# UoL-SignalProcessingGroup/SMC-NUTS

Hardware: AMD Instinct MI355X
Metric: leapfrog-steps/sec (higher is better)
Workload: dtype f64

## Files before the change

include/smcnuts_hip.h:

```cpp
#ifndef SMCNUTS_HIP_H
#define SMCNUTS_HIP_H

#include <stddef.h>
#include <stdint.h>

#ifdef __cplusplus
extern "C" {
#endif

typedef struct smcn_ctx smcn_ctx;

#define SMCN_MODEL_GAUSS 0
#define SMCN_MODEL_ARMA 1
#define SMCN_MODEL_PRMWCD 2
#define SMCN_MODEL_HOST 3
#define SMCN_MODEL_GLM 4
#define SMCN_MODEL_HGLM 5
#define SMCN_MODEL_CATEGORICAL 6
#define SMCN_MODEL_ORDINAL 7

#define SMCN_LKERNEL_FORWARD 0
#define SMCN_LKERNEL_GAUSSIAN 1

#define SMCN_FLAG_TAPE_OVERFLOW 1
// ... 17 lines not shown
int smcn_get_proposal(smcn_ctx* ctx, double* r, double* x_new, double* r_new, double* logw_new);
int smcn_set_momentum(smcn_ctx* ctx, const double* r);
int smcn_set_proposal(smcn_ctx* ctx, const double* r, const double* x_new, const double* r_new);

int smcn_target_eval(smcn_ctx* ctx, const double* x, int64_t M, double phi, double* logp,
                     double* grad, double* lpri, double* llik);
int smcn_target_constrain(smcn_ctx* ctx, const double* x, int64_t M, double* out);

int smcn_init_particles_std_normal(smcn_ctx* ctx, double phi);
int smcn_init_weights(smcn_ctx* ctx, double phi, const double* logq0);

int smcn_normalise_partials(smcn_ctx* ctx, double out[4]);
int smcn_normalise_apply(smcn_ctx* ctx, double loglik);
int smcn_normalise(smcn_ctx* ctx, double* loglik, double* ess);

int smcn_moment_sums(smcn_ctx* ctx, const double* mean_or_null, double* sums);

int smcn_resample_multinomial(smcn_ctx* ctx, const double* u, double loglik, double log_n_total,
                              int64_t iteration, int64_t* idx_out);
#define SMCN_RESAMPLE_MULTINOMIAL 0
#define SMCN_RESAMPLE_SYSTEMATIC 1
int smcn_set_resample_scheme(smcn_ctx* ctx, int scheme);
int smcn_set_wide_eval(smcn_ctx* ctx, int on);
int smcn_set_lane_grid(smcn_ctx* ctx, int64_t waves);
int smcn_set_lane_segments(smcn_ctx* ctx, int segments);

int smcn_set_nuts_cap(smcn_ctx* ctx, int doublings, int widen);
int smcn_nuts_parked(smcn_ctx* ctx, int64_t* parked);
int smcn_set_nuts_requeue(smcn_ctx* ctx, int doublings);

int smcn_propose_nuts(smcn_ctx* ctx, double step_size, double phi, int max_depth, double delta_max,
                      int64_t iteration, const double* tape, const int64_t* tape_off);
int smcn_get_tree_stats(smcn_ctx* ctx, int32_t* nleap, int32_t* depth, int32_t* ndraws, int32_t* flags);
int smcn_last_leapfrogs(smcn_ctx* ctx, int64_t* total);
int smcn_get_density_parts(smcn_ctx* ctx, double* lpri0, double* llik0, double* lpri1, double* llik1);

int smcn_reweight(smcn_ctx* ctx, int lkernel);
int smcn_accept_reject(smcn_ctx* ctx, double phi, const double* u, int64_t iteration);
int smcn_reweight_asymptotic(smcn_ctx* ctx, double phi_old, double phi_new);
int smcn_set_logw_density_ratio(smcn_ctx* ctx, double phi_num, double phi_den);

int smcn_set_lkernel_values(smcn_ctx* ctx, const double* L, const double* q);

int smcn_gauss_lkernel_sums(smcn_ctx* ctx, const double* shift, double* sums);
int smcn_gauss_lkernel_logpdf(smcn_ctx* ctx, const double* mu_x, const double* m0, const double* B,
                              const double* U, double c0);
// ... 114 lines not shown
```

smcnuts_amd/_capi.py:

```python
import ctypes as C
import os

import numpy as np

from . import build as _build

MODEL_GAUSS, MODEL_ARMA, MODEL_PRMWCD, MODEL_HOST = 0, 1, 2, 3
MODEL_GLM = 4
MODEL_HGLM = 5
MODEL_CATEGORICAL = 6
MODEL_ORDINAL = 7
HOST_TARGET_FN = C.CFUNCTYPE(C.c_int, C.c_void_p, C.c_int64, C.c_int, C.POINTER(C.c_double), C.c_int,
                             C.POINTER(C.c_double), C.POINTER(C.c_double), C.POINTER(C.c_double),
                             C.POINTER(C.c_double))
LKERNEL_FORWARD, LKERNEL_GAUSSIAN = 0, 1

_dp = C.POINTER(C.c_double)
_ip = C.POINTER(C.c_int32)
_lp = C.POINTER(C.c_int64)
_ctx = C.c_void_p

SIGNATURES = {
    "smcn_version": ([], C.c_int),
    "smcn_last_error": ([_ctx], C.c_char_p),
# ... 39 lines not shown
    "smcn_temper_partials": ([_ctx, C.c_double, C.c_double, _dp], C.c_int),
    "smcn_temper_bisect": ([_ctx, C.c_double, C.c_double, C.POINTER(C.c_double), C.POINTER(C.c_int)], C.c_int),
    "smcn_temper_bisect_pass": ([_ctx, C.c_int, C.c_double], C.c_int),
    "smcn_temper_bisect_buffers": ([_ctx, C.c_int, C.POINTER(C.c_void_p), C.POINTER(C.c_void_p)], C.c_int),
    "smcn_temper_bisect_decide": ([_ctx, C.c_int, C.c_int, C.c_double, C.c_double], C.c_int),
    "smcn_temper_bisect_result": ([_ctx, C.POINTER(C.c_double), C.POINTER(C.c_int)], C.c_int),
    "smcn_eval_proposed_parts": ([_ctx, C.c_int], C.c_int),
    "smcn_commit": ([_ctx, _lp], C.c_int),
    "smcn_fast_begin": ([_ctx, C.c_int64, C.c_int, C.c_int], C.c_int),
    "smcn_fast_buffers": ([_ctx, C.POINTER(C.c_void_p), C.POINTER(C.c_void_p), C.POINTER(C.c_int)], C.c_int),
    "smcn_set_resample_uniforms": ([_ctx, _dp], C.c_int),
    "smcn_step_begin": ([_ctx, C.c_int64], C.c_int),
    "smcn_step_finish": ([_ctx, C.c_int64, C.c_int, C.c_int, C.c_double, C.c_double, C.c_double, C.c_int,
                          C.c_double, C.c_int, C.c_int, _dp, _lp], C.c_int),
    "smcn_fast_read": ([_ctx, _dp, _dp, _dp], C.c_int),
    "smcn_fast_read_from": ([_ctx, _dp, _dp, _dp, C.c_int64], C.c_int),
    "smcn_history_download": ([_ctx, C.c_int64, C.c_int64, _dp, _dp], C.c_int),
    "smcn_fuse_begin": ([_ctx, C.c_int, C.c_int], C.c_int),
    "smcn_fuse_buffers": ([_ctx, C.POINTER(C.c_void_p), C.POINTER(C.c_void_p), C.POINTER(C.c_int)], C.c_int),
    "smcn_fuse_run": ([_ctx, C.c_int64, C.c_int, C.c_int, C.c_int, C.c_double, C.c_double, C.c_double, C.c_int,
                       C.c_double, C.c_int], C.c_int),
    "smcn_set_resample_scheme": ([_ctx, C.c_int], C.c_int),
    "smcn_set_wide_eval": ([_ctx, C.c_int], C.c_int),
    "smcn_set_lane_grid": ([_ctx, C.c_int64], C.c_int),
    "smcn_set_lane_segments": ([_ctx, C.c_int], C.c_int),
    "smcn_set_host_target": ([_ctx, HOST_TARGET_FN, C.c_void_p], C.c_int),
    "smcn_moment_sums_of": ([_ctx, _dp, C.c_int, _dp, _dp], C.c_int),
    "smcn_block_resample_local": ([_ctx, C.c_int64], C.c_int),
    "smcn_block_launch": ([_ctx, C.c_int64, C.c_int, C.c_double, C.c_double, C.c_int, C.c_double], C.c_int),
    "smcn_block_post": ([_ctx, C.c_int64, C.c_int, C.c_int], C.c_int),
    "smcn_block_partials_get": ([_ctx, C.c_int, _dp], C.c_int),
    "smcn_block_partials_set": ([_ctx, C.c_int, C.c_int, _dp], C.c_int),
    "smcn_block_stats": ([_ctx, C.c_int64, C.c_int, C.c_int, C.c_int, C.c_double, C.c_double, C.c_int], C.c_int),
    "smcn_block_wait": ([_ctx, C.c_int, C.POINTER(C.c_int), C.POINTER(C.c_int)], C.c_int),
    "smcn_block_commit": ([_ctx, C.c_int64, C.c_int], C.c_int),
    "smcn_block_ess": ([_ctx, C.c_int, _dp], C.c_int),
    "smcn_fuse_decide": ([_ctx, C.c_int64, C.c_int, C.c_int, C.c_double, C.c_double, C.POINTER(C.c_int)], C.c_int),
    "smcn_fuse_finish": ([_ctx, C.c_int64, C.c_int, C.c_int, C.c_int, C.c_double, C.c_double,
                          C.POINTER(C.c_int)], C.c_int),
    "smcn_partials_get": ([_ctx, _dp], C.c_int),
    "smcn_partials_set_gathered": ([_ctx, _dp, C.c_int], C.c_int),
    "smcn_timers": ([_ctx, _dp, C.c_int], C.c_int),
    "smcn_selftest_math": ([_ctx, _dp, C.c_int64, _dp], C.c_int),
    "smcn_measure_peaks": ([_ctx, _dp], C.c_int),
    "smcn_selftest_wide": ([_ctx, C.c_int, _dp, C.c_int64, _dp], C.c_int),
    "smcn_device_cache_trim": ([C.c_int, C.POINTER(C.c_int64), C.POINTER(C.c_int64)], C.c_int),
# ... 343 lines not shown
```

smcnuts_amd/csrc/smcn_api.hip:

```cpp
#include <hip/hip_runtime.h>

#include <dlfcn.h>

#include <cmath>
#include <cstdio>
#include <cstring>
#include <chrono>
#include <cstdlib>
#include <map>
#include <mutex>
#include <string>
#include <thread>
#include <unordered_map>
#include <vector>

#include "../../include/smcnuts_hip.h"
#include "smcn_nuts.hpp"
#include "smcn_nuts_wave.hpp"
#include "smcn_nuts_fin.hpp"
#include "smcn_nuts2.hpp"
#include "smcn_nuts3.hpp"
#include "smcn_temper.hpp"
#include "smcn_nuts_host.hpp"
#include "smcn_weights.hpp"
#include "smcn_glk.hpp"
#include "smcn_step.hpp"
#include "smcn_comm.hpp"
#include "smcn_pointwise.hpp"
#include "smcn_predict.hpp"
#include "smcn_predict_draws.hpp"

using namespace smcn;

namespace {
struct Roctx {
    int (*push)(const char*) = nullptr;
    int (*pop)() = nullptr;
    Roctx() {
        void* h = dlopen("librocprofiler-sdk-roctx.so", RTLD_LAZY | RTLD_GLOBAL);
        if (!h) h = dlopen("libroctx64.so", RTLD_LAZY | RTLD_GLOBAL);
        if (h) {
            push = (int (*)(const char*))dlsym(h, "roctxRangePushA");
            pop = (int (*)())dlsym(h, "roctxRangePop");
        }
    }
};
inline Roctx& roctx() { static Roctx r; return r; }
struct Range {
    explicit Range(const char* name) { if (roctx().push && roctx().pop) roctx().push(name); }
    ~Range() { if (roctx().push && roctx().pop) roctx().pop(); }
    Range(const Range&) = delete;
};
thread_local std::string g_create_error;
constexpr int kMaxPart = 1024;
constexpr int kTimerRing = 512;
// ... 43 lines not shown
    bool kin_valid = false;
    bool r_pm = false, r_new_pm = false;
    unsigned long long* prof = nullptr;
    double* tape_d = nullptr;
    int64_t* tape_off_d = nullptr;
    int64_t tape_cap = 0;
    bool momentum_set = false, lg_set = false, q_set = false, u_set = false;
    double *hist = nullptr, *ss = nullptr, *lp = nullptr, *gath = nullptr, *hist_x = nullptr, *hist_logw = nullptr;
    double* u_res = nullptr;
    double *in_rec = nullptr, *out_rec = nullptr;
    double* nuts_scratch = nullptr;
    int64_t nuts_scratch_len = 0;
    int64_t fast_K = -1;
    bool fast_hist = false;
    int fuse_max = 0;
    int64_t rec_cap = 0;
    int resample_scheme = 0;
    bool fused_ok = false;
    bool lane_kernel = false;
    int64_t arma_T = 0;
    double *tb_state = nullptr, *tb_part = nullptr, *tb_local = nullptr, *tb_gath = nullptr;
    int tb_world = 0, tb_blocks = 0;
    int wide_eval = 1;
    int64_t lane_grid_cap = 0;
    int lane_segments = 0;
    unsigned long long* handover = nullptr;
    int64_t handover_len = 0;
    bool plain_block = false;
    ncclComm_t comm = nullptr;
    int comm_rank = 0, comm_world = 1;
    double *g_ttot_all = nullptr, *g_toff_all = nullptr, *g_keys = nullptr, *g_keys_send = nullptr, *g_keys_recv = nullptr,
           *g_rows_send = nullptr, *g_rows_recv = nullptr;
    int32_t *g_dest = nullptr, *g_order = nullptr;
    int64_t g_serve_cap = 0;
    int g_world = 0;
    smcn_host_target_fn host_fn = nullptr;
    void* host_user = nullptr;
    double *hc_vec = nullptr, *hc_sc = nullptr, *hc_gp = nullptr, *hc_gl = nullptr;
    int32_t* hc_st = nullptr;
    std::vector<double> hx, hlp, hll, hgp, hgl;
    double* n2_ovf = nullptr;
    int64_t n2_ovf_len = 0;
    double* ss_scratch = nullptr;
    double* rows_h = nullptr;
    double* hist_h = nullptr;
    bool hist_h_valid = false;
// ... 732 lines not shown
    HIPC(c, stream_wait(c->stream));
    if (c->own_stream && c->stream) pool_give(c->device, c->stream);
    c->stream = (hipStream_t)s;
    c->own_stream = false;
    return 0;
}

int smcn_synchronize(smcn_ctx* c) {
    CHECK_CTX(c);
    HIPC(c, stream_wait(c->stream));
    return 0;
}

int smcn_set_resample_scheme(smcn_ctx* c, int scheme) {
    CHECK_CTX(c);
    if (scheme != 0 && scheme != 1) FAIL(c, "smcn_set_resample_scheme: 0 (multinomial) or 1 (systematic)");
    c->resample_scheme = scheme;
    return 0;
}
int smcn_set_wide_eval(smcn_ctx* c, int on) {
    CHECK_CTX(c);
    if (on != 0 && on != 1) FAIL(c, "smcn_set_wide_eval: 0 or 1");
    c->wide_eval = on;
    return 0;
}

int smcn_set_lane_grid(smcn_ctx* c, int64_t waves) {
    CHECK_CTX(c);
    c->lane_grid_cap = waves;
    return 0;
}

int smcn_set_lane_segments(smcn_ctx* c, int segments) {
    CHECK_CTX(c);
    if (segments < 0 || segments > 64) FAIL(c, "smcn_set_lane_segments: 0 (auto) .. 64");
    c->lane_segments = segments;
    return 0;
}

int smcn_set_host_target(smcn_ctx* c, smcn_host_target_fn fn, void* user) {
    CHECK_CTX(c);
    if (c->model != SMCN_MODEL_HOST) FAIL(c, "smcn_set_host_target: the context was not created with SMCN_MODEL_HOST");
    c->host_fn = fn;
    c->host_user = user;
    return 0;
}
// ... 784 lines not shown
        c->in_rec = c->out_rec = nullptr;
        HIPC(c, dalloc(&c->in_rec, N * cap * n2_in_doubles(D)));
        HIPC(c, dalloc(&c->out_rec, N * cap * n2_out_doubles(D)));
        c->rec_cap = cap;
    }
    const size_t lds = (size_t)n3_lds_bytes<Model>(LC, LF);
    int64_t blocks = (N + kN3Block - 1) / kN3Block;
    const int64_t resident = (int64_t)c->num_cu * 4;
    if (c->lane_grid_cap > 0 && blocks > c->lane_grid_cap) blocks = c->lane_grid_cap;
    else if (c->lane_grid_cap == 0 && blocks > resident) blocks = resident;
    if (((N + blocks - 1) / blocks + 63) / 64 > kN3ReadyWords) blocks = (N + kN3Block - 1) / kN3Block;
    if (int rc = grow_scratch(c, c->n2_ovf, c->n2_ovf_len, blocks * kN3Block * 2 * (int64_t)n3_ovf_pairs(D, LC, LF))) return rc;
    a.ovf = c->n2_ovf;
    if (phase != 2) {
        if (c->momentum_set && B != 1) FAIL(c, "nuts3: caller-supplied momenta go with single transitions");
        nuts3_prep_kernel<D><<<grid_for(N * B, 256), 256, 0, c->stream>>>(c->x, c->momentum_set ? c->r : nullptr, c->r,
                                                                         c->in_rec, N, c->base, c->seed, a.iter, B, tape_d,
                                                                         tape_off_d);
        c->momentum_set = false;
        a.in = c->in_rec;
        a.out = c->out_rec;
        a.B = B;
        a.logw0 = (fuse_reweight && B > 1) ? c->logw : nullptr;
        a.wide = (c->wide_eval ? 1 : 0) | 2;
        const bool queued = blocks * kN3Block < N;
        a.seg_len = 0;
        a.seg_tail = 0;
        a.seg_align = 4;
        if (queued) {
            const int64_t per_wave = (N + blocks - 1) / blocks, words = (per_wave + 63) / 64;
            int nseg = c->lane_segments > 0 ? c->lane_segments : 4;
            if (nseg > B) nseg = (int)B;
            while (nseg > 1 && nseg * words > kN3ReadyWords) --nseg;
            a.seg_tail = 0;
            if (nseg > 1) a.seg_len = (int)((B + nseg - 1) / nseg);
            int64_t segs = a.seg_len > 0 ? (B + a.seg_len - 1) / a.seg_len : 1;
            const int64_t last_len = B - (segs - 1) * a.seg_len;
            if (segs > 1 && last_len >= 2 && (segs + 1) * words <= kN3ReadyWords) {
                a.seg_tail = (int)((2 * last_len + 2) / 5 > 0 ? (2 * last_len + 2) / 5 : 1);
                ++segs;
            }
            const int64_t hw = N * (segs - 1) * 2 * (n2_vp(D) / 2 + 1);
            if (hw > c->handover_len) {
                HIPC(c, stream_wait(c->stream));
                if (c->handover) (void)cached_free(c->handover);
                c->handover = nullptr;
                HIPC(c, cached_malloc((void**)&c->handover, sizeof(unsigned long long) * (size_t)hw));
// ... 1966 lines not shown
```

smcnuts_amd/csrc/smcn_nuts3.hpp:

```cpp
#pragma once
#include "smcn_nuts2.hpp"
#include <type_traits>

namespace smcn {

constexpr int kN3Block = 64;
constexpr int kN3ReadyWords = 64;


__constant__ double kArmaFinishTab[24] = {
    1.4426950408889634074, 6.93147180369123816490e-01, 1.90821492927058770002e-10,
    2.08767569878680989792e-09, 2.50521083854417187751e-08, 2.75573192239858906526e-07,
    2.75573192239858906526e-06, 2.48015873015873015873e-05, 1.98412698412698412698e-04,
    1.38888888888888888889e-03, 8.33333333333333333333e-03, 4.16666666666666666667e-02,
    1.66666666666666666667e-01,
    0.70710678118654752440,
    9.52380952380952380952e-02, 1.05263157894736842105e-01, 1.17647058823529411765e-01,
    1.33333333333333333333e-01, 1.53846153846153846154e-01, 1.81818181818181818182e-01,
    2.22222222222222222222e-01, 2.85714285714285714286e-01, 4.0e-01, 6.66666666666666666667e-01};

struct ArmaLaneModel {
    static constexpr int D = 4;
    static constexpr bool HAS_WIDE = true;
    using cptr = const __attribute__((address_space(4))) double*;
// ... 186 lines not shown
        else if constexpr (A >= 8) return dpp_mov<0x110 + K>(v);
        else return dpp_mov<(K == 1) ? 0x90 : 0x44>(v);
    }
    template <int CTRL, int ROWS>
    static __device__ __forceinline__ double row_join(double v, double fill) { return dpp_fill<CTRL, ROWS>(v, fill); }
    template <class F>
    static __device__ __forceinline__ void seg_walk(const double* Yp, int S, bool extra, F&& step) {
        const int nfull = (S - 1) >> 2, rem = (S - 1) & 3;
        double yp = Yp[0];
        double c0 = Yp[1], c1 = Yp[2], c2 = Yp[3], c3 = Yp[4];
        const double* q = Yp + 5;
        for (int c = 0; c < nfull; ++c) {
            const double n0 = q[0], n1 = q[1], n2 = q[2], n3 = q[3];
            q += 4;
            step(yp, c0); step(c0, c1); step(c1, c2); step(c2, c3);
            yp = c3;
            c0 = n0; c1 = n1; c2 = n2; c3 = n3;
        }
        if (rem > 0) { step(yp, c0); yp = c0; c0 = c1; c1 = c2; c2 = c3; }
        if (rem > 1) { step(yp, c0); yp = c0; c0 = c1; c1 = c2; }
        if (rem > 2) { step(yp, c0); yp = c0; c0 = c1; }
        if (extra) step(yp, c0);
    }
    template <int A>
    __device__ __forceinline__ void recur_wide(const double (&x)[4], bool act, unsigned long long mask, const double* Yl,
                                               double __attribute__((ext_vector_type(2)))* XCH, int lane, double& ss_o,
                                               double& gm_o, double& gb_o, double& gt_o) const {
        using d2 = double __attribute__((ext_vector_type(2)));
        const int rank = (int)__builtin_amdgcn_mbcnt_hi((unsigned)(mask >> 32), __builtin_amdgcn_mbcnt_lo((unsigned)mask, 0u));
        if (act) {
            d2 t;
            t.x = x[0]; t.y = x[1];
            XCH[2 * rank] = t;
            t.x = x[2]; t.y = x[3];
            XCH[2 * rank + 1] = t;
        }
        wave_exchange_fence();
        const int g = lane / A, a = lane % A;
        const d2 q0 = XCH[2 * g], q1 = XCH[2 * g + 1];
        const double mu = q0.x, beta = q0.y, theta = q1.x;
        const double nth = -theta, nbeta = -beta;
        const int n = T - 1, S = (n + A - 1) / A, R = n - A * (S - 1);
        const bool extra = a < R;
        const int i0 = 1 + a * (S - 1) + (a < R ? a : R);
        const bool first = a == 0;
        const double y0 = Yl[0];
        const double e_init = fma(nbeta, mu, y0 - mu), dm_init = -(1.0 + beta), db_init = -mu;
        double e = first ? e_init : 0.0, dm = first ? dm_init : 0.0, db = first ? db_init : 0.0, dt = 0.0;
        auto state_step = [&](double yp, double yt) __attribute__((always_inline)) {
            dt = fma(nth, dt, -e);
            dm = fma(nth, dm, -1.0);
            db = fma(nth, db, -yp);
            e = fma(nth, e, fma(nbeta, yp, yt - mu));
        };
        seg_walk(Yl + (i0 - 1), S, extra, state_step);
        double pm = 1.0;
        {
            double base = nth;
            for (int m = S - 2; m > 0; m >>= 1) {
                pm = (m & 1) ? pm * base : pm;
                base = base * base;
            }
        }
// ... 24 lines not shown
                if constexpr (A >= 32) return dpp_mov<0x138>(v);
                else return seg_shift<A, 1>(v, 0.0);
            };
            const double ei = prev(E), mi = prev(M), bi = prev(Bv), ti = prev(Tt);
            e = first ? e_init : ei;
            dm = first ? dm_init : mi;
            db = first ? db_init : bi;
            dt = first ? 0.0 : ti;
        }
        double ss = first ? e * e : 0.0, gm = first ? e * dm : 0.0, gb = first ? e * db : 0.0, gt = 0.0;
        auto full_step = [&](double yp, double yt) __attribute__((always_inline)) {
            dt = fma(nth, dt, -e);
            dm = fma(nth, dm, -1.0);
            db = fma(nth, db, -yp);
            e = fma(nth, e, fma(nbeta, yp, yt - mu));
            ss = fma(e, e, ss);
            gm = fma(e, dm, gm);
            gb = fma(e, db, gb);
            gt = fma(e, dt, gt);
        };
        seg_walk(Yl + (i0 - 1), S, extra, full_step);
        if constexpr (A == 64) wave_sum4(ss, gm, gb, gt, ss, gm, gb, gt);
        else { ss = group_sum<A>(ss); gm = group_sum<A>(gm); gb = group_sum<A>(gb); gt = group_sum<A>(gt); }
        if (first) {
            d2 t;
            t.x = ss; t.y = gm;
            XCH[2 * g] = t;
            t.x = gb; t.y = gt;
            XCH[2 * g + 1] = t;
        }
        wave_exchange_fence();
        if (act) {
            const d2 r0 = XCH[2 * rank], r1 = XCH[2 * rank + 1];
            ss_o = r0.x; gm_o = r0.y; gb_o = r1.x; gt_o = r1.y;
        }
    }
};

template <class Model>
__global__ void __launch_bounds__(256) lane_eval_kernel(const double* mdata, const double* x, int64_t M, int64_t rs,
                                                        int64_t cs, double phi, double* logp, double* grad, int64_t grs,
                                                        int64_t gcs, double* lpri_o, double* llik_o) {
    constexpr int D = Model::D;
    Model model;
    model.init(mdata);
    for (int64_t i = (int64_t)blockIdx.x * blockDim.x + threadIdx.x; i < M; i += (int64_t)gridDim.x * blockDim.x) {
// ... 59 lines not shown

__device__ __forceinline__ bool compact_mode(const Nuts2Args& a) { return a.logw0 != nullptr; }

template <class Model, bool TAPE, int LC, int LF, bool QUEUE = false, int WPE = 1>
__global__ void __launch_bounds__(kN3Block) __attribute__((amdgpu_waves_per_eu(WPE, WPE))) nuts3_kernel(Nuts2Args a) {
    constexpr int D = Model::D, VP = n2_vp(D), VH = VP / 2;
    constexpr int INSZ = n2_in_doubles(D), OUTSZ = n2_out_doubles(D);
    constexpr int RING = 0;
    constexpr int NST = RING + 4;
    constexpr int PREF = NST + 2;
    constexpr int CAND0 = PREF + VH + 1, CREC = 2 * VH + 1;
    constexpr int FIRST0 = CAND0 + LC * CREC, FREC = 2 * VH;
    constexpr int OCAND0 = 0, OFIRST0 = (8 - LC) * CREC, OVFP = n3_ovf_pairs(D, LC, LF);
    static_assert(FIRST0 + LF * FREC == n3_lds_pairs(D, LC, LF), "LDS layout");
    static_assert(LC >= 0 && LC <= 8 && LF >= 0 && LF <= 8, "levels");
    enum { INIT = 1, LEAF = 2, DONE = 3 };

    using d2 = double __attribute__((ext_vector_type(2)));
    using gptr2 = __attribute__((address_space(1))) d2*;
    using gcptr2 = const __attribute__((address_space(1))) d2*;
    using gcptr = const __attribute__((address_space(1))) double*;
    extern __shared__ d2 lds3[];
    const int lane = (int)threadIdx.x;
    d2* const L = lds3 + lane;
    gptr2 const O = (gptr2)a.ovf + ((int64_t)blockIdx.x * OVFP) * 64 + lane;

    Model model;
    model.init(a.mdata);
    double* const Yl = reinterpret_cast<double*>(lds3 + n3_lds_pairs(D, LC, LF) * 64);
    d2* const XCH = reinterpret_cast<d2*>(Yl + (Model::HAS_WIDE ? Model::YMAX + Model::YPAD : 0));
    bool wide_ok = false, wide_rows = false;
    if constexpr (Model::HAS_WIDE) {
        wide_ok = (a.wide & 1) != 0 && model.T >= Model::WIDE_MIN_T && model.T <= Model::YMAX;
        wide_rows = wide_ok && model.T >= Model::WIDE_MIN_T_ROWS;
        if (wide_ok) {
            for (int i = lane; i < model.T + Model::YPAD; i += kN3Block) Yl[i] = i < model.T ? ((gcptr)a.mdata)[1 + i] : 0.0;
            wave_exchange_fence();
        }
    }
    const int64_t N = a.N;
    const double eps = a.eps, phi = a.phi;
    const unsigned int w_quot = (unsigned int)N / gridDim.x, w_rem = (unsigned int)N % gridDim.x;
    const unsigned int w_count = QUEUE ? w_quot + (blockIdx.x < w_rem ? 1u : 0u) : (unsigned int)kN3Block;
    const int64_t w_start = QUEUE ? (int64_t)blockIdx.x * w_quot + (blockIdx.x < w_rem ? blockIdx.x : w_rem)
                                  : (int64_t)blockIdx.x * kN3Block;
    const int64_t p_first = w_start + lane;
    const bool live = QUEUE ? (unsigned int)lane < w_count : p_first < N;
    std::conditional_t<QUEUE, int64_t, const int64_t> p = p_first;
    const int64_t pc = live ? p_first : N - 1;
    bool have_next = false, own_wait = false;
    unsigned int i_next = 0u;
    int seg_next = 0;
    unsigned int n_ready = 0u;
    double lw_next = 0.0;
    double hx_next[D];
    int64_t toff_next = 0, tlen_next = 0;
    const int Bs = (QUEUE && a.seg_len > 0) ? a.seg_len : a.B;
    const int n_main = (a.B + Bs - 1) / Bs, b_tail = (QUEUE && a.seg_tail > 0) ? a.B - a.seg_tail : a.B;
    const unsigned int nseg = (unsigned int)(n_main + (b_tail < a.B ? 1 : 0));
    auto seg_begin = [&](int sg) __attribute__((always_inline)) {
        return sg < n_main ? sg * Bs : (sg == n_main ? b_tail : a.B);
    };
    int seg = 0, b_end = seg_begin(1);
    const unsigned int w_words = (w_quot + (w_rem ? 1u : 0u) + 63u) / 64u;
    unsigned long long rm = 0ull;
#pragma unroll
    for (int k = 0; k < D; ++k) hx_next[k] = 0.0;

    auto st_vec = [&](auto ptr, const double (&v)[D]) __attribute__((always_inline)) {
#pragma unroll
        for (int k = 0; k < VH; ++k) {
            d2 t;
            t.x = v[2 * k];
            t.y = (2 * k + 1 < D) ? v[2 * k + 1 < D ? 2 * k + 1 : 0] : 0.0;
            ptr[k * 64] = t;
        }
    };
    auto ld_vec = [&](auto ptr, double (&v)[D]) __attribute__((always_inline)) {
#pragma unroll
        for (int k = 0; k < VH; ++k) {
            const d2 t = ptr[k * 64];
            v[2 * k] = t.x;
            if (2 * k + 1 < D) v[2 * k + 1 < D ? 2 * k + 1 : 0] = t.y;
        }
    };
    auto mov64 = [](double& dst, double src) __attribute__((always_inline)) {
        double t;
        asm volatile("v_mov_b64_e32 %0, %1" : "=v"(t) : "v"(src));
        dst = t;
    };
    auto movv = [&](double (&dst)[D], const double (&src)[D]) __attribute__((always_inline)) {
#pragma unroll
        for (int k = 0; k < D; ++k) mov64(dst[k], src[k]);
    };
    auto movd2 = [&](d2& dst, const d2& src) __attribute__((always_inline)) {
        double a, b;
        mov64(a, src.x);
        mov64(b, src.y);
        dst.x = a; dst.y = b;
    };
    auto with_cand = [&](int m, auto&& f) __attribute__((always_inline)) {
        if (LC == 8 || m - 2 < LC) f(L + (CAND0 + (m - 2) * CREC) * 64);
        else f(O + (OCAND0 + (m - 2 - LC) * CREC) * 64);
    };
    auto with_first = [&](int l, auto&& f) __attribute__((always_inline)) {
        if (LF == 8 || l - 3 < LF) f(L + (FIRST0 + (l - 3) * FREC) * 64);
        else f(O + (OFIRST0 + (l - 3 - LF) * FREC) * 64);
    };
    auto nst_ptr = [&](int m) __attribute__((always_inline)) -> unsigned short* {
        return reinterpret_cast<unsigned short*>(L + (NST + (m >> 3)) * 64) + (m & 7);
    };
    auto is_uturn = [](double A, double B, int dir) __attribute__((always_inline)) {
        return dir > 0 ? ((A < 0.0) || (B < 0.0)) : ((B > 0.0) || (A > 0.0));
    };

    gcptr2 const in2 = (gcptr2)a.in;
    gptr2 const out2 = (gptr2)a.out;
    constexpr int IPAIRS = INSZ / 2, OPAIRS = OUTSZ / 2;
    constexpr int CSZ2 = VH + 1;
    gcptr2 in_next = in2 + pc;
    gptr2 out_cur = compact_mode(a) ? out2 + N * OPAIRS + p : out2 + p;
    const int64_t in_stride = N * IPAIRS, out_stride = compact_mode(a) ? N * CSZ2 : N * OPAIRS;
// ... 1 lines not shown
    int phase = live ? INIT : DONE;
    double x[D], r[D], g[D];
    double ex[D], er[D], eg[D];
    double rx[D], rr[D];
    d2 rl;
    double c0x[D], c0r[D], c1x[D], c1r[D];
    d2 c0l, c1l;
    int n0 = 0, n1 = 0;
    double f1x[D], f1r[D], f2x[D], f2r[D];
    double logu = 0.0, lpri0 = 0.0, llik0 = 0.0;
    const bool compact = a.logw0 != nullptr;
    double lw = compact ? ((gcptr)a.logw0)[pc] : 0.0, k0 = 0.0;
    int j = 0, i = 0, dir = 0, n = 1, nleap = 0, b = 0;
    uint32_t q = 1, qfill = 0;
    int64_t toff = 0, tlen = 0;
    bool overflow = false;
    rl.x = rl.y = c0l.x = c0l.y = c1l.x = c1l.y = 0.0;
#pragma unroll
    for (int k = 0; k < D; ++k) {
        r[k] = g[k] = ex[k] = er[k] = eg[k] = rx[k] = rr[k] = 0.0;
        c0x[k] = c0r[k] = c1x[k] = c1r[k] = f1x[k] = f1r[k] = f2x[k] = f2r[k] = 0.0;
    }

    auto request = [&]() __attribute__((always_inline)) {
        using lptr = __attribute__((address_space(3))) void*;
        using gvptr = const __attribute__((address_space(1))) void*;
#pragma unroll
        for (int k = 0; k <= VH; ++k)
            __builtin_amdgcn_global_load_lds((gvptr)(in_next + (VH + k) * N), (lptr)(lds3 + (PREF + k) * 64), 16, 0, 0);
        in_next += in_stride;
    };
    auto take_record = [&](bool c) __attribute__((always_inline)) {
        __builtin_amdgcn_s_waitcnt(0x0F70);
        d2 pr[VH + 1];
#pragma unroll
        for (int k = 0; k <= VH; ++k) pr[k] = L[(PREF + k) * 64];
        if (c) {
#pragma unroll
            for (int k = 0; k < VH; ++k) {
                mov64(r[2 * k], pr[k].x);
                if (2 * k + 1 < D) mov64(r[2 * k + 1 < D ? 2 * k + 1 : 0], pr[k].y);
            }
            mov64(logu, pr[VH].x);
        }
        q = c ? 1u : q; qfill = c ? 0u : qfill; overflow = c ? false : overflow; nleap = c ? 0 : nleap;
        phase = c ? (int)INIT : phase;
        __builtin_amdgcn_s_waitcnt(0xC07F);
    };
    auto refill = [&]() __attribute__((always_inline)) {
        const u32x4 o = philox4x32_10({qfill >> 1, (uint32_t)(a.particle_base + p), a.iter + (uint32_t)b, kStreamNuts},
                                      (uint32_t)a.seed, (uint32_t)(a.seed >> 32));
        d2 t;
        t.x = u53(o.a, o.b);
        t.y = u53(o.c, o.d);
        L[(RING + ((qfill >> 1) & 3u)) * 64] = t;
// ... 11 lines not shown
            if ((int64_t)q < tlen) v = ((gcptr)a.tape)[toff + q];
            else { v = 0.5; overflow = true; }
        } else {
            if (q == qfill) refill();
            v = ring_read(q);
        }
        ++q;
        return v;
    };

    {
        const gcptr2 rec = in_next;
#pragma unroll
        for (int k = 0; k < VH; ++k) {
            const d2 t = rec[k * N];
            x[2 * k] = t.x;
            if (2 * k + 1 < D) x[2 * k + 1 < D ? 2 * k + 1 : 0] = t.y;
        }
        request();
        if constexpr (TAPE) {
            toff = ((const __attribute__((address_space(1))) int64_t*)a.tape_off)[pc];
            tlen = ((const __attribute__((address_space(1))) int64_t*)a.tape_off)[pc + 1] - toff;
        }
        take_record(true);
        if (a.B > 1) request();
        if (!live) phase = DONE;
    }

    if constexpr (QUEUE) {
        {
            const unsigned int wi = (unsigned int)lane, lo = wi * 64u;
            const unsigned int a0 = lo < 64u ? 64u : lo, b0 = w_count < lo + 64u ? w_count : lo + 64u;
            if (wi < w_words && b0 > a0) rm = (b0 - a0 >= 64u ? ~0ull : (1ull << (b0 - a0)) - 1ull) << (a0 - lo);
        }
        n_ready = w_count - (unsigned int)kN3Block;
    }
    PROF_DECL;
#ifdef SMCN_PROFILE
    unsigned long long iters = 0;
#endif
    auto emit_record = [&](bool last, uint32_t qdone, bool ovdone, int nldone) __attribute__((always_inline)) {
        const gptr2 orec = (compact && last) ? out2 + p : out_cur;
        out_cur += out_stride;
        d2 t;
        const unsigned long long s0 = (unsigned long long)(unsigned)nldone | ((unsigned long long)(unsigned)j << 32);
#pragma unroll
        for (int k = 0; k < VH; ++k) {
            t.x = rx[2 * k];
            t.y = (2 * k + 1 < D) ? rx[2 * k + 1 < D ? 2 * k + 1 : 0] : 0.0;
            orec[k * N] = t;
        }
        PROF(12);
        if (compact && !last) {
            double k1 = 0.0;
#pragma unroll
            for (int k = 0; k < D; ++k) k1 = fma(rr[k], rr[k], k1);
            const double cst = 0.5 * D * kLog2Pi;
            const double qk = -0.5 * k0 - cst;
            const double Lk = -0.5 * k1 - cst;
            const double c1 = combine_lp(rl.x, rl.y, 1.0);
            const double c0 = combine_lp(lpri0, llik0, 1.0);
            lw = lw + c1 - c0 + Lk - qk;
            t.x = lw;
            t.y = __longlong_as_double((long long)s0);
            orec[VH * N] = t;
        } else {
#pragma unroll
            for (int k = 0; k < VH; ++k) {
                t.x = rr[2 * k];
                t.y = (2 * k + 1 < D) ? rr[2 * k + 1 < D ? 2 * k + 1 : 0] : 0.0;
                orec[(VH + k) * N] = t;
            }
            orec[2 * VH * N] = rl;
            t.x = lpri0; t.y = llik0;
            orec[(2 * VH + 1) * N] = t;
            const unsigned long long s1 = (unsigned long long)qdone | ((unsigned long long)(ovdone ? 1u : 0u) << 32);
            t.x = __longlong_as_double((long long)s0);
            t.y = __longlong_as_double((long long)s1);
            orec[(2 * VH + 2) * N] = t;
        }
    };
    unsigned int it = 0u;
    for (;; ++it) {
        PROF(7);
        if constexpr (QUEUE) {
            if (__ballot(phase != DONE || have_next || own_wait) == 0ull && n_ready == 0u) break;
        }
        const bool act = phase != DONE;
#ifdef SMCN_PROFILE_TAIL
        PROF_ON(__popcll(__ballot(act)) <= SMCN_PROFILE_TAIL);
#endif
#ifdef SMCN_PROFILE
        if (prof_on_) ++iters;
#endif
        if constexpr (!TAPE) {
            int need = 1;
            if (phase == LEAF) {
                const int t1 = __builtin_ctz(~(unsigned)i);
                need = (t1 >= j) ? j + 2 : t1;
            }
            need = need > 7 ? 7 : need;
            const unsigned long long am0 = __ballot(act);
            const int na0 = __popcll(am0);
            if (Model::HAS_WIDE && (a.wide & 2) != 0 && na0 <= 16) {
                const int avail = (int)(qfill - q);
                if (__ballot(act && avail < (need > 2 ? need : 2)) != 0ull) {
                    using u4 = unsigned int __attribute__((ext_vector_type(4)));
                    u4* const XU = reinterpret_cast<u4*>(XCH);
                    const int rank = (int)__builtin_amdgcn_mbcnt_hi((unsigned)(am0 >> 32), __builtin_amdgcn_mbcnt_lo((unsigned)am0, 0u));
                    if (act) {
                        u4 w;
                        w.x = qfill | ((unsigned)lane << 16); w.y = q;
                        w.z = (uint32_t)(a.particle_base + p); w.w = a.iter + (uint32_t)b;
                        XU[rank] = w;
                    }
                    wave_exchange_fence();
                    const int g4 = lane >> 2, h4 = lane & 3;
                    if (g4 < na0) {
                        const u4 w = XU[g4];
                        const uint32_t oq = w.x & 0xFFFFu, ol = w.x >> 16;
                        if ((int)(oq - w.y) + 2 * (h4 + 1) <= 8) {
                            const u32x4 o = philox4x32_10({(oq >> 1) + (uint32_t)h4, w.z, w.w, kStreamNuts}, (uint32_t)a.seed,
                                                          (uint32_t)(a.seed >> 32));
                            d2 t;
                            t.x = u53(o.a, o.b);
                            t.y = u53(o.c, o.d);
                            lds3[ol + (RING + (((oq >> 1) + (uint32_t)h4) & 3u)) * 64] = t;
                        }
                    }
                    wave_exchange_fence();
                    if (act) {
                        const int nfit = (8 - avail) >> 1;
                        qfill += 2u * (uint32_t)(nfit < 0 ? 0 : (nfit > 4 ? 4 : nfit));
                    }
                }
            } else {
            if (act && (int)(qfill - q) <= 6) refill();
            for (;;) {
                const int avail = (int)(qfill - q);
                if (__ballot(act && avail < need) == 0ull) break;
                if (act && avail <= 6) refill();
            }
            }
            const uint32_t qt = q + (uint32_t)(phase == LEAF ? j : 0);
            up0 = ring_read(q); up1 = ring_read(q + 1u);
            utop = ring_read(qt); udir = ring_read(phase == LEAF ? qt + 1u : qt);
            pre_ok = (int)(qfill - qt) > 1;
        }
        PROF(0);

        const double e = dir * eps, h = dir * eps / 2;
        if (phase == LEAF) {
#pragma unroll
            for (int k = 0; k < D; ++k) r[k] = r[k] + h * g[k];
#pragma unroll
            for (int k = 0; k < D; ++k) x[k] = x[k] + e * r[k];
        }
        double lpri = 0.0, llik = 0.0, gp[D], gl[D];
#pragma unroll
        for (int k = 0; k < D; ++k) { gp[k] = 0.0; gl[k] = 0.0; }
        PROF(1);
        if constexpr (Model::HAS_WIDE) {
            const unsigned long long amask = __ballot(act);
            const int nact = __popcll(amask);
            double ss = 0.0, gm = 0.0, gb = 0.0, gt = 0.0;
            if (!wide_ok || nact > 16) {
                if (act) model.recur(x, ss, gm, gb, gt);
            } else if (nact > 8) model.template recur_wide<4>(x, act, amask, Yl, XCH, lane, ss, gm, gb, gt);
            else if (nact > 4) model.template recur_wide<8>(x, act, amask, Yl, XCH, lane, ss, gm, gb, gt);
            else if (nact > 2 || !wide_rows) model.template recur_wide<16>(x, act, amask, Yl, XCH, lane, ss, gm, gb, gt);
            else if (nact == 2) model.template recur_wide<32>(x, act, amask, Yl, XCH, lane, ss, gm, gb, gt);
            else model.template recur_wide<64>(x, act, amask, Yl, XCH, lane, ss, gm, gb, gt);
            if (act) model.finish(x, ss, gm, gb, gt, lpri, llik, gp, gl);
        } else {
            if (act) model.eval(x, lpri, llik, gp, gl);
        }
        PROF(2);
        double lp = lpri + phi * llik;
#pragma unroll
        for (int k = 0; k < D; ++k) g[k] = fma(phi, gl[k], gp[k]);
        if (!finite_d(lp)) {
            mov64(lp, -kInf);
#pragma unroll
            for (int k = 0; k < D; ++k) mov64(g[k], -kInf);
        }
// ... 1 lines not shown
        bool start_doubling = false;
        bool tree_end = false;
        const bool init = phase == INIT;
        if (phase == LEAF) {
            double kin = 0.0;
#pragma unroll
            for (int k = 0; k < D; ++k) r[k] = r[k] + h * g[k];
#pragma unroll
            for (int k = 0; k < D; ++k) kin = fma(r[k], r[k], kin);
            ++nleap;
            const double joint = lp - 0.5 * kin;
            int nsub = (logu < joint) ? 1 : 0;
            bool ssub = (logu - a.delta_max) >= joint;
            d2 leafl;
            leafl.x = lpri; leafl.y = llik;
            {
                const bool opens = j > 0 && (i & 1) == 0;
                const int lopen = opens ? ((i == 0) ? j : (__ffs(i) - 1)) : 0;
                if (lopen >= 1) {
                    movv(f1x, x); movv(f1r, r);
                    if (lopen >= 2) { movv(f2x, x); movv(f2r, r); }
                }
                for (int l = 3; l <= lopen; ++l)
                    with_first(l, [&](auto fp) __attribute__((always_inline)) { st_vec(fp, x); st_vec(fp + VH * 64, r); });
            }
            int csrc = -1;
            auto cand_value = [&](bool need, double (&cx)[D], double (&cr)[D], d2& cl) __attribute__((always_inline)) {
#pragma unroll
                for (int k = 0; k < D; ++k) { cx[k] = x[k]; cr[k] = r[k]; }
                cl = leafl;
                if (need && csrc >= 0) {
                    if (csrc == 0) { movv(cx, c0x); movv(cr, c0r); movd2(cl, c0l); }
                    else if (csrc == 1) { movv(cx, c1x); movv(cr, c1r); movd2(cl, c1l); }
                    else with_cand(csrc, [&](auto cp) __attribute__((always_inline)) {
                        double tx[D], tr[D];
                        ld_vec(cp, tx); ld_vec(cp + VH * 64, tr);
                        const d2 tl = cp[2 * VH * 64];
                        movv(cx, tx); movv(cr, tr); movd2(cl, tl);
                    });
                }
            };
            auto merge = [&](int m, double u, int nfirst, const double (&fx)[D], const double (&fr)[D]) __attribute__((always_inline)) {
                const int den = (nfirst + nsub) > 1 ? (nfirst + nsub) : 1;
                const bool keep = !(fma(u, (double)den, -(double)nsub) < 0.0);
                csrc = keep ? m : csrc;
                nsub += nfirst;
                double A = 0.0, B = 0.0;
// ... 43 lines not shown
                double u;
                if (TAPE || !pre_ok) u = ring_draw(); else { u = utop; ++q; }
                acc = nsub >= n || fma(u, (double)n, -(double)nsub) < 0.0;
                double A = 0.0, B = 0.0;
#pragma unroll
                for (int k = 0; k < D; ++k) {
                    const double d = x[k] - ex[k];
                    A = fma(d, er[k], A);
                    B = fma(d, r[k], B);
                }
                stop = is_uturn(A, B, dir);
                done = true;
            }
            PROF(9);
            {
                double cx[D], cr[D];
                d2 cl;
                const bool park = how == 3;
                cand_value(park || acc, cx, cr, cl);
                if (acc) { movv(rx, cx); movv(rr, cr); movd2(rl, cl); }
                if (park) {
                    if (m == 0) { movv(c0x, cx); movv(c0r, cr); movd2(c0l, cl); }
                    else if (m == 1) { movv(c1x, cx); movv(c1r, cr); movd2(c1l, cl); }
                    else {
                        with_cand(m, [&](auto crec) __attribute__((always_inline)) { st_vec(crec, cx); st_vec(crec + VH * 64, cr); crec[2 * VH * 64] = cl; });
                        *nst_ptr(m) = (unsigned short)nsub;
                    }
                }
                n0 = (park && m == 0) ? nsub : n0;
                n1 = (park && m == 1) ? nsub : n1;
            }
            PROF(4);
            if (!done) {
                ++i;
            } else {
                n += nsub;
                ++j;
                if (stop || j > a.max_depth) {
                    if constexpr (QUEUE) {
                        tree_end = true;
                    } else {
                        const bool more = b + 1 < a.B;
                        const int bdone = b;
                        const uint32_t qdone = q;
                        const bool ovdone = overflow;
                        const int nldone = nleap;
                        if (more) movv(x, rx);
                        phase = DONE;
                        take_record(more);
                        b = more ? bdone + 1 : b;
                        PROF(10);
                        emit_record(!more, qdone, ovdone, nldone);
                        PROF(13);
                        if (more && bdone + 2 < a.B) request();
                    }
                } else {
                    start_doubling = true;
                }
            }
        }
        if constexpr (QUEUE) {
            if (__ballot(tree_end || (phase == DONE && (have_next || own_wait || n_ready != 0u))) != 0ull) {
                __builtin_amdgcn_s_waitcnt(0x0F70);
                const bool idle = phase == DONE;
                const bool sd = b + 1 >= b_end;
                const bool last = tree_end && b + 1 >= a.B;
                const bool in_step = ((it + 1u) & (unsigned int)(a.seg_align - 1)) == 0u;
                const bool to_next = have_next && ((tree_end && sd) || idle);
                const bool take = to_next && in_step;
                const bool push = tree_end && have_next && sd && !last;
                const bool to_own = (tree_end && !(have_next && sd) && !last) || (idle && own_wait);
                const bool cont = to_own && in_step;
                own_wait = to_own && !in_step;
                const bool seg_done = cont && sd;
                const int bdone = b;
                const uint32_t qdone = q;
                const bool ovdone = overflow;
// ... 104 lines not shown
            phase = init ? (int)LEAF : phase;
        }
        PROF(5);
        {
            int nd = dir;
            if (start_doubling) {
                double u;
                if (TAPE || !pre_ok) u = ring_draw(); else { u = udir; ++q; }
                nd = (u < 0.5) ? 1 : -1;
            }
            const bool first = start_doubling && dir == 0;
            const bool swap = start_doubling && dir != 0 && nd != dir;
            if (first || swap) {
                double tx[D], tr[D], tg[D];
#pragma unroll
                for (int k = 0; k < D; ++k) { tx[k] = ex[k]; tr[k] = er[k]; tg[k] = eg[k]; }
                movv(ex, x); movv(er, r); movv(eg, g);
                if (swap) { movv(x, tx); movv(r, tr); movv(g, tg); }
            }
            dir = nd;
            i = start_doubling ? 0 : i;
        }
        PROF(6);
        if constexpr (!QUEUE) {
            if (__ballot(phase != DONE) == 0ull) break;
        }
    }
    PROF_FLUSH(a);
#ifdef SMCN_PROFILE
    if (lane == 0) {
        atomicAdd(&a.prof[14], iters);
        atomicMax(&a.prof[15], iters);
    }
#endif
}

}
```

Measured before the change: 7.731 billion.

## Add solo mode: whole wavefront cooperates on last remaining NUTS particle

When only one lane in a wavefront still has an unfinished NUTS trajectory, the kernel broadcasts that lane's full state to all lanes with readlane and continues in a solo loop. Every lane then redundantly runs the tree logic while the wide likelihood recursion splits the time series across all 64 lanes without the LDS exchange. Only the owner lane performs stores, and RNG refill is spread across lanes. This targets the tail where a single long trajectory leaves 63 lanes idle, at the cost of a large state broadcast, more code size and register pressure, and a new default-on path.

Result: no change. 7.686 billion (-0.6%).

```diff
diff --git a/include/smcnuts_hip.h b/include/smcnuts_hip.h
--- a/include/smcnuts_hip.h
+++ b/include/smcnuts_hip.h
@@ -63,6 +63,7 @@
 #define SMCN_RESAMPLE_SYSTEMATIC 1
 int smcn_set_resample_scheme(smcn_ctx* ctx, int scheme);
 int smcn_set_wide_eval(smcn_ctx* ctx, int on);
+int smcn_set_lane_solo(smcn_ctx* ctx, int on);
 int smcn_set_lane_grid(smcn_ctx* ctx, int64_t waves);
 int smcn_set_lane_segments(smcn_ctx* ctx, int segments);
 
diff --git a/smcnuts_amd/_capi.py b/smcnuts_amd/_capi.py
--- a/smcnuts_amd/_capi.py
+++ b/smcnuts_amd/_capi.py
@@ -85,6 +85,7 @@
                        C.c_double, C.c_int], C.c_int),
     "smcn_set_resample_scheme": ([_ctx, C.c_int], C.c_int),
     "smcn_set_wide_eval": ([_ctx, C.c_int], C.c_int),
+    "smcn_set_lane_solo": ([_ctx, C.c_int], C.c_int),
     "smcn_set_lane_grid": ([_ctx, C.c_int64], C.c_int),
     "smcn_set_lane_segments": ([_ctx, C.c_int], C.c_int),
     "smcn_set_host_target": ([_ctx, HOST_TARGET_FN, C.c_void_p], C.c_int),
diff --git a/smcnuts_amd/csrc/smcn_api.hip b/smcnuts_amd/csrc/smcn_api.hip
--- a/smcnuts_amd/csrc/smcn_api.hip
+++ b/smcnuts_amd/csrc/smcn_api.hip
@@ -31,6 +31,10 @@
 #include "smcn_predict_draws.hpp"
 
 using namespace smcn;
+
+#ifndef SMCN_LANE_SOLO_DEFAULT
+#define SMCN_LANE_SOLO_DEFAULT 1
+#endif
 
 namespace {
 struct Roctx {
@@ -120,6 +124,7 @@
     double *tb_state = nullptr, *tb_part = nullptr, *tb_local = nullptr, *tb_gath = nullptr;
     int tb_world = 0, tb_blocks = 0;
     int wide_eval = 1;
+    int lane_solo = SMCN_LANE_SOLO_DEFAULT;
     int64_t lane_grid_cap = 0;
     int lane_segments = 0;
     unsigned long long* handover = nullptr;
@@ -898,6 +903,12 @@
     CHECK_CTX(c);
     if (on != 0 && on != 1) FAIL(c, "smcn_set_wide_eval: 0 or 1");
     c->wide_eval = on;
+    return 0;
+}
+int smcn_set_lane_solo(smcn_ctx* c, int on) {
+    CHECK_CTX(c);
+    if (on != 0 && on != 1) FAIL(c, "smcn_set_lane_solo: 0 or 1");
+    c->lane_solo = on;
     return 0;
 }
 
@@ -1728,7 +1739,7 @@
         a.out = c->out_rec;
         a.B = B;
         a.logw0 = (fuse_reweight && B > 1) ? c->logw : nullptr;
-        a.wide = (c->wide_eval ? 1 : 0) | 2;
+        a.wide = (c->wide_eval ? 1 : 0) | 2 | (c->lane_solo ? 4 : 0);
         const bool queued = blocks * kN3Block < N;
         a.seg_len = 0;
         a.seg_tail = 0;
diff --git a/smcnuts_amd/csrc/smcn_nuts3.hpp b/smcnuts_amd/csrc/smcn_nuts3.hpp
--- a/smcnuts_amd/csrc/smcn_nuts3.hpp
+++ b/smcnuts_amd/csrc/smcn_nuts3.hpp
@@ -232,23 +232,29 @@
         if (rem > 2) { step(yp, c0); yp = c0; c0 = c1; }
         if (extra) step(yp, c0);
     }
-    template <int A>
+    template <int A, bool SHARED = false>
     __device__ __forceinline__ void recur_wide(const double (&x)[4], bool act, unsigned long long mask, const double* Yl,
                                                double __attribute__((ext_vector_type(2)))* XCH, int lane, double& ss_o,
                                                double& gm_o, double& gb_o, double& gt_o) const {
         using d2 = double __attribute__((ext_vector_type(2)));
+        static_assert(!SHARED || A == 64, "one particle, the whole wavefront");
         const int rank = (int)__builtin_amdgcn_mbcnt_hi((unsigned)(mask >> 32), __builtin_amdgcn_mbcnt_lo((unsigned)mask, 0u));
-        if (act) {
-            d2 t;
-            t.x = x[0]; t.y = x[1];
-            XCH[2 * rank] = t;
-            t.x = x[2]; t.y = x[3];
-            XCH[2 * rank + 1] = t;
-        }
-        wave_exchange_fence();
         const int g = lane / A, a = lane % A;
-        const d2 q0 = XCH[2 * g], q1 = XCH[2 * g + 1];
-        const double mu = q0.x, beta = q0.y, theta = q1.x;
+        double mu, beta, theta;
+        if constexpr (SHARED) {
+            mu = x[0]; beta = x[1]; theta = x[2];
+        } else {
+            if (act) {
+                d2 t;
+                t.x = x[0]; t.y = x[1];
+                XCH[2 * rank] = t;
+                t.x = x[2]; t.y = x[3];
+                XCH[2 * rank + 1] = t;
+            }
+            wave_exchange_fence();
+            const d2 q0 = XCH[2 * g], q1 = XCH[2 * g + 1];
+            mu = q0.x; beta = q0.y; theta = q1.x;
+        }
         const double nth = -theta, nbeta = -beta;
         const int n = T - 1, S = (n + A - 1) / A, R = n - A * (S - 1);
         const bool extra = a < R;
@@ -319,6 +325,10 @@
         seg_walk(Yl + (i0 - 1), S, extra, full_step);
         if constexpr (A == 64) wave_sum4(ss, gm, gb, gt, ss, gm, gb, gt);
         else { ss = group_sum<A>(ss); gm = group_sum<A>(gm); gb = group_sum<A>(gb); gt = group_sum<A>(gt); }
+        if constexpr (SHARED) {
+            ss_o = ss; gm_o = gm; gb_o = gb; gt_o = gt;
+            return;
+        }
         if (first) {
             d2 t;
             t.x = ss; t.y = gm;
@@ -424,8 +434,8 @@
     using gcptr = const __attribute__((address_space(1))) double*;
     extern __shared__ d2 lds3[];
     const int lane = (int)threadIdx.x;
-    d2* const L = lds3 + lane;
-    gptr2 const O = (gptr2)a.ovf + ((int64_t)blockIdx.x * OVFP) * 64 + lane;
+    d2* L = lds3 + lane;
+    gptr2 O = (gptr2)a.ovf + ((int64_t)blockIdx.x * OVFP) * 64 + lane;
 
     Model model;
     model.init(a.mdata);
@@ -448,7 +458,7 @@
                                   : (int64_t)blockIdx.x * kN3Block;
     const int64_t p_first = w_start + lane;
     const bool live = QUEUE ? (unsigned int)lane < w_count : p_first < N;
-    std::conditional_t<QUEUE, int64_t, const int64_t> p = p_first;
+    int64_t p = p_first;
     const int64_t pc = live ? p_first : N - 1;
     bool have_next = false, own_wait = false;
     unsigned int i_next = 0u;
@@ -486,20 +496,10 @@
             if (2 * k + 1 < D) v[2 * k + 1 < D ? 2 * k + 1 : 0] = t.y;
         }
     };
-    auto mov64 = [](double& dst, double src) __attribute__((always_inline)) {
+    auto mov64_lane = [](double& dst, double src) __attribute__((always_inline)) {
         double t;
         asm volatile("v_mov_b64_e32 %0, %1" : "=v"(t) : "v"(src));
         dst = t;
-    };
-    auto movv = [&](double (&dst)[D], const double (&src)[D]) __attribute__((always_inline)) {
-#pragma unroll
-        for (int k = 0; k < D; ++k) mov64(dst[k], src[k]);
-    };
-    auto movd2 = [&](d2& dst, const d2& src) __attribute__((always_inline)) {
-        double a, b;
-        mov64(a, src.x);
-        mov64(b, src.y);
-        dst.x = a; dst.y = b;
     };
     auto with_cand = [&](int m, auto&& f) __attribute__((always_inline)) {
         if (LC == 8 || m - 2 < LC) f(L + (CAND0 + (m - 2) * CREC) * 64);
@@ -547,15 +547,17 @@
         c0x[k] = c0r[k] = c1x[k] = c1r[k] = f1x[k] = f1r[k] = f2x[k] = f2r[k] = 0.0;
     }
 
-    auto request = [&]() __attribute__((always_inline)) {
+    auto request = [&](bool ld = true) __attribute__((always_inline)) {
         using lptr = __attribute__((address_space(3))) void*;
         using gvptr = const __attribute__((address_space(1))) void*;
-#pragma unroll
-        for (int k = 0; k <= VH; ++k)
-            __builtin_amdgcn_global_load_lds((gvptr)(in_next + (VH + k) * N), (lptr)(lds3 + (PREF + k) * 64), 16, 0, 0);
+        if (ld) {
+#pragma unroll
+            for (int k = 0; k <= VH; ++k)
+                __builtin_amdgcn_global_load_lds((gvptr)(in_next + (VH + k) * N), (lptr)(lds3 + (PREF + k) * 64), 16, 0, 0);
+        }
         in_next += in_stride;
     };
-    auto take_record = [&](bool c) __attribute__((always_inline)) {
+    auto take_record_with = [&](bool c, auto&& mov64) __attribute__((always_inline)) {
         __builtin_amdgcn_s_waitcnt(0x0F70);
         d2 pr[VH + 1];
 #pragma unroll
@@ -613,7 +615,7 @@
             toff = ((const __attribute__((address_space(1))) int64_t*)a.tape_off)[pc];
             tlen = ((const __attribute__((address_space(1))) int64_t*)a.tape_off)[pc + 1] - toff;
         }
-        take_record(true);
+        take_record_with(true, mov64_lane);
         if (a.B > 1) request();
         if (!live) phase = DONE;
     }
@@ -630,16 +632,18 @@
 #ifdef SMCN_PROFILE
     unsigned long long iters = 0;
 #endif
-    auto emit_record = [&](bool last, uint32_t qdone, bool ovdone, int nldone) __attribute__((always_inline)) {
+    auto emit_record = [&](bool last, uint32_t qdone, bool ovdone, int nldone, bool wr = true) __attribute__((always_inline)) {
         const gptr2 orec = (compact && last) ? out2 + p : out_cur;
         out_cur += out_stride;
         d2 t;
         const unsigned long long s0 = (unsigned long long)(unsigned)nldone | ((unsigned long long)(unsigned)j << 32);
-#pragma unroll
-        for (int k = 0; k < VH; ++k) {
-            t.x = rx[2 * k];
-            t.y = (2 * k + 1 < D) ? rx[2 * k + 1 < D ? 2 * k + 1 : 0] : 0.0;
-            orec[k * N] = t;
+        if (wr) {
+#pragma unroll
+            for (int k = 0; k < VH; ++k) {
+                t.x = rx[2 * k];
+                t.y = (2 * k + 1 < D) ? rx[2 * k + 1 < D ? 2 * k + 1 : 0] : 0.0;
+                orec[k * N] = t;
+            }
         }
         PROF(12);
         if (compact && !last) {
@@ -654,8 +658,8 @@
             lw = lw + c1 - c0 + Lk - qk;
             t.x = lw;
             t.y = __longlong_as_double((long long)s0);
-            orec[VH * N] = t;
-        } else {
+            if (wr) orec[VH * N] = t;
+        } else if (wr) {
 #pragma unroll
             for (int k = 0; k < VH; ++k) {
                 t.x = rr[2 * k];
@@ -672,14 +676,34 @@
         }
     };
     unsigned int it = 0u;
-    for (;; ++it) {
+    constexpr bool CAN_SOLO = !QUEUE && !TAPE && Model::HAS_WIDE;
+    const bool solo_on = CAN_SOLO && wide_rows && (a.wide & 4) != 0;
+    int owner = 0;
+    auto iteration = [&](auto solo_c) __attribute__((always_inline)) -> int {
+        constexpr bool SOLO = decltype(solo_c)::value;
+        const bool own = !SOLO || lane == owner;
+        auto mov64 = [&](double& dst, double src) __attribute__((always_inline)) {
+            if constexpr (SOLO) dst = src;
+            else mov64_lane(dst, src);
+        };
+        auto movv = [&](double (&dst)[D], const double (&src)[D]) __attribute__((always_inline)) {
+#pragma unroll
+            for (int k = 0; k < D; ++k) mov64(dst[k], src[k]);
+        };
+        auto movd2 = [&](d2& dst, const d2& src) __attribute__((always_inline)) {
+            double a, b;
+            mov64(a, src.x);
+            mov64(b, src.y);
+            dst.x = a; dst.y = b;
+        };
+        auto take_record = [&](bool c) __attribute__((always_inline)) { take_record_with(c, mov64); };
         PROF(7);
         if constexpr (QUEUE) {
-            if (__ballot(phase != DONE || have_next || own_wait) == 0ull && n_ready == 0u) break;
-        }
-        const bool act = phase != DONE;
+            if (__ballot(phase != DONE || have_next || own_wait) == 0ull && n_ready == 0u) return 0;
+        }
+        const bool act = SOLO || phase != DONE;
 #ifdef SMCN_PROFILE_TAIL
-        PROF_ON(__popcll(__ballot(act)) <= SMCN_PROFILE_TAIL);
+        PROF_ON(SOLO || __popcll(__ballot(act)) <= SMCN_PROFILE_TAIL);
 #endif
 #ifdef SMCN_PROFILE
         if (prof_on_) ++iters;
@@ -691,6 +715,23 @@
                 need = (t1 >= j) ? j + 2 : t1;
             }
             need = need > 7 ? 7 : need;
+            if constexpr (SOLO) {
+                const int avail = (int)(qfill - q);
+                if (avail < (need > 2 ? need : 2)) {
+                    if (lane < 4 && avail + 2 * (lane + 1) <= 8) {
+                        const uint32_t blk = (qfill >> 1) + (uint32_t)lane;
+                        const u32x4 o = philox4x32_10({blk, (uint32_t)(a.particle_base + p), a.iter + (uint32_t)b, kStreamNuts},
+                                                      (uint32_t)a.seed, (uint32_t)(a.seed >> 32));
+                        d2 t;
+                        t.x = u53(o.a, o.b);
+                        t.y = u53(o.c, o.d);
+                        L[(RING + (blk & 3u)) * 64] = t;
+                    }
+                    wave_exchange_fence();
+                    const int nfit = (8 - avail) >> 1;
+                    qfill += 2u * (uint32_t)(nfit < 0 ? 0 : (nfit > 4 ? 4 : nfit));
+                }
+            } else {
             const unsigned long long am0 = __ballot(act);
             const int na0 = __popcll(am0);
             if (Model::HAS_WIDE && (a.wide & 2) != 0 && na0 <= 16) {
@@ -733,6 +774,7 @@
                 if (act && avail <= 6) refill();
             }
             }
+            }
             const uint32_t qt = q + (uint32_t)(phase == LEAF ? j : 0);
             up0 = ring_read(q); up1 = ring_read(q + 1u);
             utop = ring_read(qt); udir = ring_read(phase == LEAF ? qt + 1u : qt);
@@ -751,7 +793,11 @@
 #pragma unroll
         for (int k = 0; k < D; ++k) { gp[k] = 0.0; gl[k] = 0.0; }
         PROF(1);
-        if constexpr (Model::HAS_WIDE) {
+        if constexpr (SOLO) {
+            double ss = 0.0, gm = 0.0, gb = 0.0, gt = 0.0;
+            model.template recur_wide<64, true>(x, true, ~0ull, Yl, XCH, lane, ss, gm, gb, gt);
+            model.finish(x, ss, gm, gb, gt, lpri, llik, gp, gl);
+        } else if constexpr (Model::HAS_WIDE) {
             const unsigned long long amask = __ballot(act);
             const int nact = __popcll(amask);
             double ss = 0.0, gm = 0.0, gb = 0.0, gt = 0.0;
@@ -799,7 +845,7 @@
                     if (lopen >= 2) { movv(f2x, x); movv(f2r, r); }
                 }
                 for (int l = 3; l <= lopen; ++l)
-                    with_first(l, [&](auto fp) __attribute__((always_inline)) { st_vec(fp, x); st_vec(fp + VH * 64, r); });
+                    if (own) with_first(l, [&](auto fp) __attribute__((always_inline)) { st_vec(fp, x); st_vec(fp + VH * 64, r); });
             }
             int csrc = -1;
             auto cand_value = [&](bool need, double (&cx)[D], double (&cr)[D], d2& cl) __attribute__((always_inline)) {
@@ -889,7 +935,7 @@
                 if (park) {
                     if (m == 0) { movv(c0x, cx); movv(c0r, cr); movd2(c0l, cl); }
                     else if (m == 1) { movv(c1x, cx); movv(c1r, cr); movd2(c1l, cl); }
-                    else {
+                    else if (own) {
                         with_cand(m, [&](auto crec) __attribute__((always_inline)) { st_vec(crec, cx); st_vec(crec + VH * 64, cr); crec[2 * VH * 64] = cl; });
                         *nst_ptr(m) = (unsigned short)nsub;
                     }
@@ -917,9 +963,9 @@
                         take_record(more);
                         b = more ? bdone + 1 : b;
                         PROF(10);
-                        emit_record(!more, qdone, ovdone, nldone);
+                        emit_record(!more, qdone, ovdone, nldone, own);
                         PROF(13);
-                        if (more && bdone + 2 < a.B) request();
+                        if (more && bdone + 2 < a.B) request(own);
                     }
                 } else {
                     start_doubling = true;
@@ -1070,8 +1116,55 @@
             i = start_doubling ? 0 : i;
         }
         PROF(6);
-        if constexpr (!QUEUE) {
-            if (__ballot(phase != DONE) == 0ull) break;
+        if constexpr (SOLO) return phase != DONE ? 1 : 0;
+        else if constexpr (!QUEUE) return __popcll(__ballot(phase != DONE));
+        else return 64;
+    };
+    bool go_solo = solo_on && __popcll(__ballot(phase != DONE)) == 1;
+    if (!go_solo) {
+        for (;; ++it) {
+            const int left = iteration(std::false_type{});
+            if (left == 0) break;
+            if constexpr (CAN_SOLO) {
+                if (left == 1 && solo_on) { go_solo = true; break; }
+            }
+        }
+    }
+    if constexpr (CAN_SOLO) {
+        if (go_solo) {
+            owner = __builtin_amdgcn_readfirstlane((int)__builtin_ctzll(__ballot(phase != DONE)));
+            auto bi = [&](auto& v) __attribute__((always_inline)) { v = (std::remove_reference_t<decltype(v)>)__builtin_amdgcn_readlane((int)v, owner); };
+            auto bd = [&](double& v) __attribute__((always_inline)) {
+                v = __hiloint2double(__builtin_amdgcn_readlane(__double2hiint(v), owner), __builtin_amdgcn_readlane(__double2loint(v), owner));
+            };
+            auto bl = [&](unsigned long long v) __attribute__((always_inline)) -> unsigned long long {
+                const unsigned int lo = (unsigned int)__builtin_amdgcn_readlane((int)(unsigned int)v, owner);
+                const unsigned int hi = (unsigned int)__builtin_amdgcn_readlane((int)(unsigned int)(v >> 32), owner);
+                return ((unsigned long long)hi << 32) | lo;
+            };
+            auto bv = [&](double (&v)[D]) __attribute__((always_inline)) {
+#pragma unroll
+                for (int k = 0; k < D; ++k) bd(v[k]);
+            };
+            auto b2 = [&](d2& v) __attribute__((always_inline)) {
+                double a0 = v.x, a1 = v.y;
+                bd(a0); bd(a1);
+                v.x = a0; v.y = a1;
+            };
+            bv(x); bv(r); bv(g); bv(ex); bv(er); bv(eg); bv(rx); bv(rr); b2(rl);
+            bv(c0x); bv(c0r); bv(c1x); bv(c1r); b2(c0l); b2(c1l); bi(n0); bi(n1);
+            bv(f1x); bv(f1r); bv(f2x); bv(f2r);
+            bd(logu); bd(lpri0); bd(llik0); bd(lw); bd(k0);
+            bi(j); bi(i); bi(dir); bi(n); bi(nleap); bi(b); bi(q); bi(qfill); bi(phase);
+            overflow = __builtin_amdgcn_readlane((int)overflow, owner) != 0;
+            p = (int64_t)bl((unsigned long long)p);
+            in_next = (gcptr2)bl((unsigned long long)in_next);
+            out_cur = (gptr2)bl((unsigned long long)out_cur);
+            L = lds3 + owner;
+            O = (gptr2)a.ovf + ((int64_t)blockIdx.x * OVFP) * 64 + owner;
+            for (;;) {
+                if (iteration(std::true_type{}) == 0) break;
+            }
         }
     }
     PROF_FLUSH(a);
```
